# wcy199705/DfFintheWild

Hardware: AMD Instinct MI355X
Metric: focal-stacks/sec (10x3x256x256) (higher is better)
Workload: dtype bf16x3 (split-bf16 MFMA operands hi+lo, fp32 accumulate, fp32-accurate); 1 GPU; DFF_net forward, 10-slice 3x256x256 focal stacks, batch 32 per GPU (BASELINE.json config 3), dense focus_dists, synthetic weights seed 0; batch_per_gpu=32, global_batch=32, slices=10, height=256, width=256, parallelism=single GPU, precision=bf16x3, input=float32 (B,3,N,H,W), the reference's tensor contract

## Files before the change

### dffinthewild_amd/csrc/dffw_conv_rollx.hip

```cpp
#include <algorithm>
#include <cstdio>
#include <cstdlib>
#include <utility>

#include "dffw_conv_roll.h"
#include "dffw_device.h"
#include "dffw_persist.h"

namespace dffw {

namespace rollx {
constexpr int TY = 8, TX = 16, FY = TY + 2, FX = TX + 2, HALF = FX / 2, NW = 4, RING = 6;
constexpr int ROWE = 2 * FX;
constexpr int TPL = 6144;
constexpr int SLOTB = 2 * TPL;
constexpr int PPW = 3;
constexpr int NCH = 18;
static_assert(FY * ROWE * 16 <= TPL && TPL % 1024 == 0 && 2 * (TPL / 1024) == NW * PPW, "piece layout");
static_assert((2 * ROWE) % 16 == 8, "a wave's two rows must be 8 bank groups apart");
}

template <bool RELU, int ABL = 0, bool NTS = false>
__global__ __launch_bounds__(256) __attribute__((amdgpu_waves_per_eu(2, 2))) void conv_rollx_pair(const ConvArgs a, const RollArgs t) {
    using namespace rollx;
    __shared__ __attribute__((aligned(1024))) unsigned char smem[RING * SLOTB];

    const int lane = threadIdx.x & 63;
    const int wave = __builtin_amdgcn_readfirstlane(threadIdx.x >> 6);
    const int g = lane >> 4, r = lane & 15;

    const UnitRange ur = persistent_range(t.total_tiles);
    const int ufirst = ur.first, uend = ur.end, wgs_per_xcd = ur.step;
    if (ufirst >= uend) return;
    using Unit = RollUnit;
    auto decode = [&](int u) { return roll_unit<TY, TX>(u, t, a.No); };

    const bool two = a.C1 != 0;
    const int tsel = wave >> 1;
    const int recb = two ? 32 : 64;
    const char *tbase = reinterpret_cast<const char *>((two && tsel) ? a.in1 : a.in0) + (two ? 0 : tsel * 16);
    const int slice_bytes = a.Hi * a.Wi * recb;
    int fyx[PPW], foff[PPW];
#pragma unroll
    for (int k = 0; k < PPW; ++k) {
        const int e = ((wave & 1) * PPW + k) * 64 + lane;
        const int fy = e / ROWE, j = e - fy * ROWE;
        const int part = j >= FX ? 1 : 0, sx = j - part * FX;
        const int fx = sx < HALF ? 2 * sx : 2 * (sx - HALF) + 1;
        fyx[k] = fy | (fx << 8) | (e < FY * ROWE ? 0 : 1 << 16);
        foff[k] = (fy * a.Wi + fx) * recb + part * (recb / 2);
    }
    int fvo[PPW];
    const char *fbase = tbase;
    int fu = ufirst, fq = 0, fslices = 0, fz = 0;
    auto setup_fill = [&]() {
        const Unit c = decode(fu);
        fslices = c.nz + 2;
        fz = c.zbeg - 1;
        fbase = tbase + ((int64_t)c.b * a.Ni * a.Hi * a.Wi + (int64_t)(c.gy0 - 1) * a.Wi + (c.gx0 - 1)) * recb;
#pragma unroll
        for (int k = 0; k < PPW; ++k) {
            const int iy = c.gy0 - 1 + (fyx[k] & 0xFF), ix = c.gx0 - 1 + ((fyx[k] >> 8) & 0xFF);
            fvo[k] = (!(fyx[k] >> 16) && (unsigned)iy < (unsigned)a.Hi && (unsigned)ix < (unsigned)a.Wi) ? foff[k] : (int)0x80000000;
        }
    };
    setup_fill();
    int fslotb = 0;
    auto issue_piece = [&](auto K) {
        constexpr int k = decltype(K)::value;
        const bool zin = (unsigned)fz < (unsigned)a.Ni && fu < uend;
        const auto rs = __builtin_amdgcn_make_buffer_rsrc(const_cast<char *>(fbase), 0, zin ? (int)0x80000000 : 0, 0x00020000);
        __builtin_amdgcn_raw_ptr_buffer_load_lds(rs, (__attribute__((address_space(3))) void *)(smem + fslotb + (wave * PPW + k) * 1024), 16, fvo[k],
                                                 zin ? fz * slice_bytes : 0, 0, 0);
    };
    auto advance_fill = [&]() {
        fslotb = (fslotb + SLOTB == RING * SLOTB) ? 0 : fslotb + SLOTB;
        ++fz;
        if (++fq == fslices && fu < uend) {
            fq = 0;
            fu += wgs_per_xcd;
            if (fu < uend) setup_fill();
        }
    };
#pragma unroll
    for (int q = 0; q < RING - 1; ++q) {
        issue_piece(std::integral_constant<int, 0>{});
        issue_piece(std::integral_constant<int, 1>{});
        issue_piece(std::integral_constant<int, 2>{});
        advance_fill();
    }

    const int rr = r >> 3, pp = r & 7;
    const int prow = (wave & 1) + 4 * (wave >> 1) + 2 * rr, pcol = 2 * pp + (g >> 1);
    const unsigned lds0 = (unsigned)(uintptr_t)(__attribute__((address_space(3))) unsigned char *)smem;
    const unsigned lbase = lds0 + (g & 1) * TPL + (prow * ROWE + (g >> 1) * HALF + pp) * 16;
    const int vob = ((prow * a.Wo + pcol) * 16 + (g & 1) * 8) * 2;

    short8 w[NCH][2];
    {
        const short8 *wp = reinterpret_cast<const short8 *>(t.wroll) + lane;
#pragma unroll
        for (int c = 0; c < NCH; ++c) {
            w[c][0] = wp[(c * 2 + 0) * 64];
            w[c][1] = wp[(c * 2 + 1) * 64];
        }
    }
    const f32x4 bias4 = *reinterpret_cast<const f32x4 *>(a.bias + (g & 1) * 4);
    __builtin_amdgcn_s_waitcnt(0x0F70);
    asm volatile("s_barrier" ::: "memory");

    int sidxb = 0;
    f32x4 acc0 = bias4, acc1 = {0.f, 0.f, 0.f, 0.f}, acc2 = {0.f, 0.f, 0.f, 0.f};
    char *pptr = nullptr;
    StepTrace trc(a.trace, wave, lane, NW);

    auto step = [&](auto LIVE_, auto PEND_, auto PEND2_, char *optr) {
        constexpr bool LIVE = decltype(LIVE_)::value, PEND = decltype(PEND_)::value, PEND2 = decltype(PEND2_)::value;
        trc.stamp(0);
        float v0 = 0.f, v1 = 0.f, v2 = 0.f, v3 = 0.f;
        uint32_t h01 = 0, h23 = 0, l01 = 0, l23 = 0;
        if constexpr (PEND) {
            v0 = acc0[0] + (acc1[0] + acc2[0]);
            v1 = acc0[1] + (acc1[1] + acc2[1]);
            v2 = acc0[2] + (acc1[2] + acc2[2]);
            v3 = acc0[3] + (acc1[3] + acc2[3]);
            if constexpr (RELU) {
                v0 = relu_bits(v0);
                v1 = relu_bits(v1);
                v2 = relu_bits(v2);
                v3 = relu_bits(v3);
            }
        }
        auto side = [&](auto S) {
            constexpr int s = decltype(S)::value;
            typedef __attribute__((ext_vector_type(2))) float f2;
            typedef __attribute__((ext_vector_type(2))) __bf16 b2;
            if constexpr (PEND && s == 0) {
                h01 = __builtin_bit_cast(uint32_t, __builtin_convertvector(f2{v0, v1}, b2));
                h23 = __builtin_bit_cast(uint32_t, __builtin_convertvector(f2{v2, v3}, b2));
            }
            if constexpr (PEND && s == 1) {
                v0 -= __uint_as_float(h01 << 16);
                v1 -= __uint_as_float(h01 & 0xFFFF0000u);
                v2 -= __uint_as_float(h23 << 16);
                v3 -= __uint_as_float(h23 & 0xFFFF0000u);
            }
            if constexpr (PEND && s == 2) {
                l01 = __builtin_bit_cast(uint32_t, __builtin_convertvector(f2{v0, v1}, b2));
                l23 = __builtin_bit_cast(uint32_t, __builtin_convertvector(f2{v2, v3}, b2));
            }
            if constexpr (PEND && s == 3) swap16(h01, l01);
            if constexpr (PEND && s == 4) swap16(h23, l23);
            if constexpr (PEND && s == 5 && !(ABL & 8)) {
                typedef unsigned u32x4 __attribute__((ext_vector_type(4)));
                u32x4 *dst = reinterpret_cast<u32x4 *>(pptr + (uint32_t)vob);
                if constexpr (NTS) __builtin_nontemporal_store(u32x4{h01, h23, l01, l23}, dst);
                else *dst = u32x4{h01, h23, l01, l23};
            }
            if constexpr (PEND && s == 5 && (ABL & 8)) asm volatile("" ::"v"(h01), "v"(h23), "v"(l01), "v"(l23));
            if constexpr (s == 6 && !(ABL & 4)) issue_piece(std::integral_constant<int, 0>{});
            if constexpr (s == 7 && !(ABL & 4)) issue_piece(std::integral_constant<int, 1>{});
            if constexpr (s == 8 && !(ABL & 4)) issue_piece(std::integral_constant<int, 2>{});
        };
        if constexpr (LIVE) {
            unsigned ad[3];
            {
                int sb = sidxb;
                ad[0] = lbase + sb;
                sb = (sb + SLOTB == RING * SLOTB) ? 0 : sb + SLOTB;
                ad[1] = lbase + sb;
                sb = (sb + SLOTB == RING * SLOTB) ? 0 : sb + SLOTB;
                ad[2] = lbase + sb;
            }
            trc.stamp(1);
            constexpr int DEPTH = 2, NB = DEPTH + 1;
            short8 x[NB][2];
            auto fetch = [](auto C, short8 (&xx)[NB][2], const unsigned (&adr)[3]) {
                constexpr int c = decltype(C)::value;
                constexpr int imm = (((c % 6) / 2) * ROWE + (c % 2)) * 16;
                asm volatile("ds_read_b128 %0, %1 offset:%2" : "=v"(xx[c % NB][0]) : "v"(adr[c / 6]), "n"(imm));
                asm volatile("ds_read_b128 %0, %1 offset:%2" : "=v"(xx[c % NB][1]) : "v"(adr[c / 6]), "n"(imm + FX * 16));
            };
            if constexpr (!(ABL & 1)) static_for<DEPTH>([&](auto C) { fetch(C, x, ad); });
            else static_for<NB>([&](auto C) { x[decltype(C)::value][0] = w[0][0]; x[decltype(C)::value][1] = w[1][1]; });
            f32x4 n0 = bias4, n1 = {0.f, 0.f, 0.f, 0.f}, n2 = {0.f, 0.f, 0.f, 0.f};
            static_for<NCH>([&](auto C) {
                constexpr int c = decltype(C)::value;
                if constexpr (c + DEPTH < NCH && !(ABL & 1)) fetch(std::integral_constant<int, c + DEPTH>{}, x, ad);
                constexpr int ahead = (NCH - 1 - c < DEPTH ? NCH - 1 - c : DEPTH) * 2;
                if constexpr (!(ABL & 1)) asm volatile("s_waitcnt lgkmcnt(%2)" : "+v"(x[c % NB][0]), "+v"(x[c % NB][1]) : "n"(ahead));
                else asm volatile("" : "+v"(x[c % NB][0]), "+v"(x[c % NB][1]));
                if constexpr (!(ABL & 2)) {
                    n0 = mma<false>(w[c][0], x[c % NB][0], n0);
                    n1 = mma<false>(w[c][1], x[c % NB][0], n1);
                    n2 = mma<false>(w[c][0], x[c % NB][1], n2);
                } else {
                    asm volatile("" ::"v"(x[c % NB][0]), "v"(x[c % NB][1]), "v"(w[c][0]), "v"(w[c][1]));
                }
                __builtin_amdgcn_sched_barrier(0);
                if constexpr (c >= 1 && c <= 9) {
                    side(std::integral_constant<int, c - 1>{});
                    __builtin_amdgcn_sched_barrier(0);
                }
            });
            acc0 = n0;
            acc1 = n1;
            acc2 = n2;
        } else {
            static_for<9>([&](auto S) { side(S); });
        }
        trc.stamp(2);
        constexpr int INFLIGHT = 2 * PPW + (PEND ? 1 : 0) + (PEND2 ? 1 : 0);
        if constexpr (!(ABL & 16)) asm volatile("s_waitcnt vmcnt(%0)\n\ts_barrier" ::"n"(INFLIGHT) : "memory");
        else asm volatile("s_waitcnt vmcnt(%0)" ::"n"(INFLIGHT) : "memory");
        trc.stamp(3);
        sidxb = (sidxb + SLOTB == RING * SLOTB) ? 0 : sidxb + SLOTB;
        advance_fill();
        pptr = optr;
        trc.stamp(4);
        trc.next();
    };

    int hist = 0;
    auto dispatch = [&](bool live, char *optr) {
        using T = std::true_type;
        using F = std::false_type;
        switch ((live ? 4 : 0) | hist) {
            case 0: step(F{}, F{}, F{}, optr); break;
            case 1: step(F{}, T{}, F{}, optr); break;
            case 2: step(F{}, F{}, T{}, optr); break;
            case 3: step(F{}, T{}, T{}, optr); break;
            case 4: step(T{}, F{}, F{}, optr); break;
            case 5: step(T{}, T{}, F{}, optr); break;
            case 6: step(T{}, F{}, T{}, optr); break;
            default: step(T{}, T{}, T{}, optr); break;
        }
        hist = ((hist << 1) & 2) | (live ? 1 : 0);
    };

    const int64_t ostride = (int64_t)a.Ho * a.Wo * 32;
    for (int cu = ufirst; cu < uend; cu += wgs_per_xcd) {
        const Unit U = decode(cu);
        char *optr = reinterpret_cast<char *>(a.out) + ((((int64_t)U.b * a.No + U.zbeg) * a.Ho + U.gy0) * a.Wo + U.gx0) * 32;
        for (int st = 0; st < U.nz + 2; ++st) {
            dispatch(st < U.nz, optr);
            optr += ostride;
        }
    }
    asm volatile("s_waitcnt vmcnt(0)" ::: "memory");
}

namespace rollk2 {
constexpr int TY = 8, TX = 16, FY = TY + 2, FX = TX + 2, NW = 8, RING = 5;
constexpr int ROWE = 4 * FX;
constexpr int ROWB = ROWE * 16;
constexpr int PARTB = 2 * FX * 16;
constexpr int HPL = 12 * 1024;
constexpr int SLOTB = 2 * HPL;
constexpr int PPW = 3;
constexpr int NCH = 15;
constexpr int XCH_OFF = RING * SLOTB, XCHB = 8 * 1024;
static_assert(FY * ROWB <= HPL && 2 * (HPL / 1024) == NW * PPW, "piece layout");
}

template <bool RELU>
__global__ __launch_bounds__(512) __attribute__((amdgpu_waves_per_eu(2, 2))) void conv_rollx_k2(const ConvArgs a, const RollArgs t) {
    using namespace rollk2;
    __shared__ __attribute__((aligned(1024))) unsigned char smem[XCH_OFF + 2 * XCHB];

    const int lane = threadIdx.x & 63;
    const int wave = __builtin_amdgcn_readfirstlane(threadIdx.x >> 6);
    const int half = wave >> 2, wq = wave & 3;
    const int g = lane >> 4, r = lane & 15;

    const UnitRange ur = persistent_range(t.total_tiles);
    const int ufirst = ur.first, uend = ur.end, wgs_per_xcd = ur.step;
    if (ufirst >= uend) return;
    using Unit = RollUnit;
    auto decode = [&](int u) { return roll_unit<TY, TX>(u, t, a.No); };

    const bool two = a.C1 != 0;
    const int recb = two ? 64 : 128;
    const char *tbase = reinterpret_cast<const char *>((two && half) ? a.in1 : a.in0) + (two ? 0 : half * 32);
    const int slice_bytes = a.Hi * a.Wi * recb;
    int fyx[PPW], foff[PPW];
#pragma unroll
    for (int k = 0; k < PPW; ++k) {
        const int e = (wq * PPW + k) * 64 + lane;
        const int fy = e / ROWE, j = e - fy * ROWE;
        const int part = j >= 2 * FX ? 1 : 0, q = j - part * 2 * FX;
        const int fx = q >> 1, oct = q & 1;
        fyx[k] = fy | (fx << 8) | (e < FY * ROWE ? 0 : 1 << 16);
        foff[k] = (fy * a.Wi + fx) * recb + part * (recb / 2) + oct * 16;
    }
    int fvo[PPW];
    const char *fbase = tbase;
    int fu = ufirst, fq = 0, fslices = 0, fz = 0;
    auto setup_fill = [&]() {
        const Unit c = decode(fu);
        fslices = c.nz + 2;
        fz = c.zbeg - 1;
        fbase = tbase + ((int64_t)c.b * a.Ni * a.Hi * a.Wi + (int64_t)(c.gy0 - 1) * a.Wi + (c.gx0 - 1)) * recb;
#pragma unroll
        for (int k = 0; k < PPW; ++k) {
            const int iy = c.gy0 - 1 + (fyx[k] & 0xFF), ix = c.gx0 - 1 + ((fyx[k] >> 8) & 0xFF);
            fvo[k] = (!(fyx[k] >> 16) && (unsigned)iy < (unsigned)a.Hi && (unsigned)ix < (unsigned)a.Wi) ? foff[k] : (int)0x80000000;
        }
    };
    setup_fill();
    int fslotb = 0;
    auto issue_piece = [&](auto K) {
        constexpr int k = decltype(K)::value;
        const bool zin = (unsigned)fz < (unsigned)a.Ni && fu < uend;
        const auto rs = __builtin_amdgcn_make_buffer_rsrc(const_cast<char *>(fbase), 0, zin ? (int)0x80000000 : 0, 0x00020000);
        __builtin_amdgcn_raw_ptr_buffer_load_lds(rs, (__attribute__((address_space(3))) void *)(smem + fslotb + (wave * PPW + k) * 1024), 16, fvo[k],
                                                 zin ? fz * slice_bytes : 0, 0, 0);
    };
    auto advance_fill = [&]() {
        fslotb = (fslotb + SLOTB == RING * SLOTB) ? 0 : fslotb + SLOTB;
        ++fz;
        if (++fq == fslices && fu < uend) {
            fq = 0;
            fu += wgs_per_xcd;
            if (fu < uend) setup_fill();
        }
    };
#pragma unroll
    for (int q = 0; q < RING - 1; ++q) {
        issue_piece(std::integral_constant<int, 0>{});
        issue_piece(std::integral_constant<int, 1>{});
        issue_piece(std::integral_constant<int, 2>{});
        advance_fill();
    }

    const unsigned lds0 = (unsigned)(uintptr_t)(__attribute__((address_space(3))) unsigned char *)smem;
    unsigned aoff[5];
#pragma unroll
    for (int k5 = 0; k5 < 5; ++k5) {
        const int tap9 = 2 * k5 + (g >> 1);
        const int dy = tap9 < 9 ? tap9 / 3 : 0, dx = tap9 < 9 ? tap9 % 3 : 0;
        aoff[k5] = lds0 + half * HPL + (2 * wq + dy) * ROWB + ((r + dx) * 2 + (g & 1)) * 16;
    }
    const int myrow = 2 * wq + half;
    const int vob = ((myrow * a.Wo + r) * 32 + (g & 1) * 16 + (g >> 1) * 8) * 2;
    const unsigned xch_wr = lds0 + XCH_OFF + ((2 * wq + (half ^ 1)) * 64 + lane) * 16;
    const unsigned xch_rd = lds0 + XCH_OFF + (myrow * 64 + lane) * 16;

    short8 w[NCH][2];
    {
        const short8 *wp = reinterpret_cast<const short8 *>(t.wroll) + (size_t)half * NCH * 2 * 64 + lane;
#pragma unroll
        for (int c = 0; c < NCH; ++c) {
            w[c][0] = wp[(c * 2 + 0) * 64];
            w[c][1] = wp[(c * 2 + 1) * 64];
        }
    }
    f32x4 bias4 = *reinterpret_cast<const f32x4 *>(a.bias + g * 4);
    if (half) bias4 = f32x4{0.f, 0.f, 0.f, 0.f};
    __builtin_amdgcn_s_waitcnt(0x0F70);
    asm volatile("s_barrier" ::: "memory");

    int sidxb = 0, xpar = 0;
    f32x4 mine = {0.f, 0.f, 0.f, 0.f};
    char *pptr = nullptr;

    auto step = [&](auto LIVE_, auto PEND_, auto PEND2_, char *optr) {
        constexpr bool LIVE = decltype(LIVE_)::value, PEND = decltype(PEND_)::value, PEND2 = decltype(PEND2_)::value;
        float v0 = 0.f, v1 = 0.f, v2 = 0.f, v3 = 0.f;
        uint32_t h01 = 0, h23 = 0, l01 = 0, l23 = 0;
        f32x4 theirs = {0.f, 0.f, 0.f, 0.f};
        if constexpr (PEND) {
            const unsigned ad = xch_rd + (xpar ^ 1) * XCHB;
            asm volatile("ds_read_b128 %0, %1" : "=v"(theirs) : "v"(ad));
            if constexpr (!LIVE) asm volatile("s_waitcnt lgkmcnt(0)" : "+v"(theirs));
        }
        auto side = [&](auto S) {
            constexpr int s = decltype(S)::value;
            typedef __attribute__((ext_vector_type(2))) float f2;
            typedef __attribute__((ext_vector_type(2))) __bf16 b2;
            if constexpr (PEND && s == 0) {
                v0 = mine[0] + theirs[0];
                v1 = mine[1] + theirs[1];
                v2 = mine[2] + theirs[2];
                v3 = mine[3] + theirs[3];
                if constexpr (RELU) {
                    v0 = relu_bits(v0);
                    v1 = relu_bits(v1);
                    v2 = relu_bits(v2);
                    v3 = relu_bits(v3);
                }
            }
            if constexpr (PEND && s == 1) {
                h01 = __builtin_bit_cast(uint32_t, __builtin_convertvector(f2{v0, v1}, b2));
                h23 = __builtin_bit_cast(uint32_t, __builtin_convertvector(f2{v2, v3}, b2));
            }
            if constexpr (PEND && s == 2) {
                v0 -= __uint_as_float(h01 << 16);
                v1 -= __uint_as_float(h01 & 0xFFFF0000u);
                v2 -= __uint_as_float(h23 << 16);
                v3 -= __uint_as_float(h23 & 0xFFFF0000u);
            }
            if constexpr (PEND && s == 3) {
                l01 = __builtin_bit_cast(uint32_t, __builtin_convertvector(f2{v0, v1}, b2));
                l23 = __builtin_bit_cast(uint32_t, __builtin_convertvector(f2{v2, v3}, b2));
            }
            if constexpr (PEND && s == 4) swap16(h01, l01);
            if constexpr (PEND && s == 5) swap16(h23, l23);
            if constexpr (PEND && s == 6) {
                typedef unsigned u32x4 __attribute__((ext_vector_type(4)));
                *reinterpret_cast<u32x4 *>(pptr + (uint32_t)vob) = u32x4{h01, h23, l01, l23};
            }
            if constexpr (s == 7) issue_piece(std::integral_constant<int, 0>{});
            if constexpr (s == 8) issue_piece(std::integral_constant<int, 1>{});
            if constexpr (s == 9) issue_piece(std::integral_constant<int, 2>{});
        };
        if constexpr (LIVE) {
            int sb[3];
            sb[0] = sidxb;
            sb[1] = (sb[0] + SLOTB == RING * SLOTB) ? 0 : sb[0] + SLOTB;
            sb[2] = (sb[1] + SLOTB == RING * SLOTB) ? 0 : sb[1] + SLOTB;
            constexpr int DEPTH = 2, NB = DEPTH + 1;
            short8 x[NB][2][2];
            auto fetch = [](auto C, short8 (&xx)[NB][2][2], const unsigned (&ao)[5], const int (&sbb)[3]) {
                constexpr int c = decltype(C)::value;
                const unsigned ad = ao[c % 5] + sbb[c / 5];
                asm volatile("ds_read_b128 %0, %1" : "=v"(xx[c % NB][0][0]) : "v"(ad));
                asm volatile("ds_read_b128 %0, %1 offset:%2" : "=v"(xx[c % NB][0][1]) : "v"(ad), "n"(PARTB));
                asm volatile("ds_read_b128 %0, %1 offset:%2" : "=v"(xx[c % NB][1][0]) : "v"(ad), "n"(ROWB));
                asm volatile("ds_read_b128 %0, %1 offset:%2" : "=v"(xx[c % NB][1][1]) : "v"(ad), "n"(ROWB + PARTB));
            };
            static_for<DEPTH>([&](auto C) { fetch(C, x, aoff, sb); });
            f32x4 n[2][3];
#pragma unroll
            for (int j = 0; j < 2; ++j) {
                n[j][0] = bias4;
                n[j][1] = f32x4{0.f, 0.f, 0.f, 0.f};
                n[j][2] = f32x4{0.f, 0.f, 0.f, 0.f};
            }
            static_for<NCH>([&](auto C) {
                constexpr int c = decltype(C)::value;
                if constexpr (c + DEPTH < NCH) fetch(std::integral_constant<int, c + DEPTH>{}, x, aoff, sb);
                constexpr int ahead = (NCH - 1 - c < DEPTH ? NCH - 1 - c : DEPTH) * 4;
                asm volatile("s_waitcnt lgkmcnt(%4)" : "+v"(x[c % NB][0][0]), "+v"(x[c % NB][0][1]), "+v"(x[c % NB][1][0]), "+v"(x[c % NB][1][1]) : "n"(ahead));
                if constexpr (PEND && c == 0) asm volatile("" : "+v"(theirs));
#pragma unroll
                for (int j = 0; j < 2; ++j) {
                    n[j][0] = mma<false>(w[c][0], x[c % NB][j][0], n[j][0]);
                    n[j][1] = mma<false>(w[c][1], x[c % NB][j][0], n[j][1]);
                    n[j][2] = mma<false>(w[c][0], x[c % NB][j][1], n[j][2]);
                }
                __builtin_amdgcn_sched_barrier(0);
                if constexpr (c >= 1 && c <= 10) {
                    side(std::integral_constant<int, c - 1>{});
                    __builtin_amdgcn_sched_barrier(0);
                }
            });
            f32x4 give;
#pragma unroll
            for (int i = 0; i < 4; ++i) {
                const float s0 = n[0][0][i] + (n[0][1][i] + n[0][2][i]), s1 = n[1][0][i] + (n[1][1][i] + n[1][2][i]);
                mine[i] = half ? s1 : s0;
                give[i] = half ? s0 : s1;
            }
            const unsigned wad = xch_wr + xpar * XCHB;
            asm volatile("ds_write_b128 %0, %1" ::"v"(wad), "v"(give) : "memory");
        } else {
            static_for<10>([&](auto S) { side(S); });
        }
        constexpr int INFLIGHT = PPW + (PEND ? 1 : 0);
        asm volatile("s_waitcnt vmcnt(%0) lgkmcnt(0)\n\ts_barrier" ::"n"(INFLIGHT) : "memory");
        (void)PEND2;
        sidxb = (sidxb + SLOTB == RING * SLOTB) ? 0 : sidxb + SLOTB;
        xpar ^= 1;
        advance_fill();
        pptr = optr;
    };

    int hist = 0;
    auto dispatch = [&](bool live, char *optr) {
        using T = std::true_type;
        using F = std::false_type;
        switch ((live ? 2 : 0) | (hist & 1)) {
            case 0: step(F{}, F{}, F{}, optr); break;
            case 1: step(F{}, T{}, F{}, optr); break;
            case 2: step(T{}, F{}, F{}, optr); break;
            default: step(T{}, T{}, F{}, optr); break;
        }
        hist = live ? 1 : 0;
    };

    const int64_t ostride = (int64_t)a.Ho * a.Wo * 64;
    for (int cu = ufirst; cu < uend; cu += wgs_per_xcd) {
        const Unit U = decode(cu);
        char *optr = reinterpret_cast<char *>(a.out) + ((((int64_t)U.b * a.No + U.zbeg) * a.Ho + U.gy0) * a.Wo + U.gx0) * 64;
        for (int st = 0; st < U.nz + 2; ++st) {
            dispatch(st < U.nz, optr);
            optr += ostride;
        }
    }
    asm volatile("s_waitcnt vmcnt(0)" ::: "memory");
}

bool rollx_k2_ok(int prec, const ConvArgs &a) {
    if (prec != P_BF16X3 || (a.dbg & DFFW_ARGS_NO_ROLLX)) return false;
    if (!a.out || a.out_pre || a.outf || a.res0 || a.res1 || a.res_bcast || a.cls_w || a.relu == 2 || a.Cout != 16) return false;
    if (!((a.C0 == 32 && a.C1 == 0) || (a.C0 == 16 && a.C1 == 16))) return false;
    const int64_t recb = a.C1 ? 64 : 128;
    return (int64_t)(a.Ni + 1) * a.Hi * a.Wi * recb < (1ll << 31);
}

static const RollRow kRollxK2[] = {DFFW_ROW(rollk2::NW * 64, conv_rollx_k2, false), DFFW_ROW(rollk2::NW * 64, conv_rollx_k2, true)};
hipError_t launch_conv_rollx_k2(const ConvArgs &a, const RollArgs &t, hipStream_t s) {
    return launch_row(&kRollxK2[a.relu == 1], t.total_tiles, t.wgs > 0 ? t.wgs : 256, 1, s, a, t);
}
void conv_rollx_k2_kernel_name(const ConvArgs &a, char *buf, int n) { copy_row_name(&kRollxK2[a.relu == 1], buf, n); }

bool rollx_pair_ok(int prec, const ConvArgs &a, bool pair) {
    if (prec != P_BF16X3 || !pair || (a.dbg & DFFW_ARGS_NO_ROLLX)) return false;
    if (!a.out || a.out_pre || a.outf || a.res0 || a.res1 || a.res_bcast || a.cls_w || a.relu == 2 || a.Cout != 8) return false;
    if (!((a.C0 == 16 && a.C1 == 0) || (a.C0 == 8 && a.C1 == 8))) return false;
    const int64_t recb = a.C1 ? 32 : 64;
    return (int64_t)(a.Ni + 1) * a.Hi * a.Wi * recb < (1ll << 31);
}

static const RollRow kRollxPair[] = {
    {"dffw::conv_rollx_pair<false>", conv_rollx_pair<false>, rollx::NW * 64},
    {"dffw::conv_rollx_pair<true>", conv_rollx_pair<true>, rollx::NW * 64},
#ifdef DFFW_ABL_BUILD
    DFFW_ROW(rollx::NW * 64, conv_rollx_pair, true, 3, false), DFFW_ROW(rollx::NW * 64, conv_rollx_pair, true, 12, false),
    DFFW_ROW(rollx::NW * 64, conv_rollx_pair, true, 0, true),
#endif
};
// ... 17 lines not shown
```

### dffinthewild_amd/csrc/dffw_ops.cpp

```cpp
#include <functional>
#include <string>
#include <vector>

#include "dffw_bn.h"
#include "dffw_conv_pw_wgrad.h"
#include "dffw_conv_wgrad.h"
#include "dffw_pool_grad.h"
#include "dffw_run.h"
#include "dffw_score_grad.h"
#include "dffw_stem_wgrad.h"

using namespace dffw;

namespace {

struct OpEngine : dffw_engine {
    OpEngine(int device_, int prec_) { device = device_; prec = prec_; }
};

struct OpBlock {
    char *p = nullptr;
    hipStream_t s;
    explicit OpBlock(hipStream_t s_) : s(s_) {}
    OpBlock(const OpBlock &) = delete;
// ... 82 lines not shown
    return dffw_op_conv3d_ex(device, precision, x, B, Cin, N, H, W, weight, Cout, kernel, stride, pad, dilation, transposed, bn, conv_bias, residual, relu, y,
                             nullptr, nullptr, nullptr, hip_stream);
}

int dffw_op_conv3d_ex(int device, int precision, const float *x, int B, int Cin, int N, int H, int W, const float *weight,
                      int Cout, const int kernel[3], const int stride[3], const int pad[3], const int dilation[3], int transposed,
                      const float *bn, const float *conv_bias, const float *residual, int relu, float *y, float *y_pre, const float *cls_weight,
                      float *cls_score, void *hip_stream) {
    if (!x || !weight || !y || !kernel || !stride || !pad || !dilation) return fail(DFFW_EINVAL, "null argument");
    if (precision < 0 || precision > 2) return fail(DFFW_EINVAL, "unknown precision %d", precision);
    if (stride[0] != 1 || dilation[0] != 1) return fail(DFFW_EINVAL, "slice stride/dilation must be 1");
    if (stride[1] != stride[2] || dilation[1] != dilation[2]) return fail(DFFW_EINVAL, "row/col stride and dilation must match");
    if (Cout != 1 && Cout % 4) return fail(DFFW_EINVAL, "Cout must be 1 or a multiple of 4");
    if (Cout > 128) return fail(DFFW_EINVAL, "Cout > 128 unsupported");
    HIPCHK(hipSetDevice(device));
    LayerDef L{"op", "", Cin, Cout, kernel[0], kernel[1], kernel[2], stride[1], stride[2], pad[0], pad[1], pad[2],
               dilation[1], dilation[2], transposed != 0, true, false};
    if (transposed && !(kernel[0] == 3 && kernel[1] == 3 && kernel[2] == 3 && stride[1] == 2 && pad[0] == 1 && pad[1] == 1 && pad[2] == 1))
        return fail(DFFW_EINVAL, "transposed conv supports only k3 s(1,2,2) p1 op(0,1,1)");
    OpEngine eng(device, precision);
    int rc = pack_conv(L, precision, weight, bn, conv_bias, eng.convs["op"]);
    if (rc) return rc;
    if ((cls_weight != nullptr) != (cls_score != nullptr)) return fail(DFFW_EINVAL, "cls_weight and cls_score go together");
    if ((y_pre || cls_weight) && (Cout == 1 || Cout % 8)) return fail(DFFW_EINVAL, "second output / fused classifier need Cout %% 8 == 0");
    if (cls_weight) {
        LayerDef C{"cls", "", Cout, 1, 1, 1, 1, 1, 1, 0, 0, 0, 1, 1, false, true, false};
        rc = pack_conv(C, precision, cls_weight, nullptr, nullptr, eng.convs["cls"]);
        if (rc) return rc;
    }
    const int cpad = (Cin + 7) / 8 * 8;
    const bool stem = (!transposed && kernel[0] == 1 && kernel[1] == 9 && kernel[2] == 9 && dilation[1] == 2 && pad[0] == 0 && pad[1] == 8 &&
                       stride[1] == 1 && Cin == 3);
    return run_op(eng, (hipStream_t)hip_stream, false, [&](Run &r) {
        Act in = r.act(B, N, H, stem ? W + 2 : W, cpad);
        const int64_t plane = (int64_t)N * H * W;
        float *xp = !stem && cpad != Cin ? (float *)r.raw(B * cpad * plane * (int64_t)sizeof(float)) : nullptr;
        if (real(r)) {
            if (stem || xp) r.check(hipMemsetAsync(in.p, 0, (size_t)in.pixels() * prec_parts(precision) * cpad * 2, r.s), "input memset");
            if (stem) {
                r.check(launch_stack_in(precision, x, in.p, B, N, H, W, r.s), "stack_in");
            } else if (!xp) {
                r.check(launch_from_ncdhw(precision, x, in.p, B, Cin, N, H, W, r.s), "from_ncdhw");
            } else {
                r.check(hipMemsetAsync(xp, 0, (size_t)B * cpad * plane * sizeof(float), r.s), "input memset");
                for (int b = 0; b < B && r.ok(); ++b)
                    r.check(hipMemcpyAsync(xp + (int64_t)b * cpad * plane, x + (int64_t)b * Cin * plane, (size_t)Cin * plane * sizeof(float),
                                           hipMemcpyDeviceToDevice, r.s), "copy");
                if (r.ok()) r.check(launch_from_ncdhw(precision, xp, in.p, B, cpad, N, H, W, r.s), "from_ncdhw");
            }
        }
        const int No = N + 2 * pad[0] - (kernel[0] - 1);
        const int Ho = transposed ? 2 * H : (H + 2 * pad[1] - dilation[1] * (kernel[1] - 1) - 1) / stride[1] + 1;
        const int Wo = transposed ? 2 * W : (W + 2 * pad[2] - dilation[2] * (kernel[2] - 1) - 1) / stride[2] + 1;
        const int64_t opix = (int64_t)B * No * Ho * Wo;
        ConvOpt o;
        o.relu = relu;
        Act res, pre;
        if (Cout == 1) {
            o.outf = (float *)r.raw(opix * sizeof(float));
        } else if (residual) {
            res = stage_in(r, residual, B, Cout, No, Ho, Wo);
            o.res0 = &res;
        }
        if (y_pre) o.out_pre = &pre;
        if (cls_weight) {
            o.cls = "cls";
            o.cls_out = (float *)r.raw(opix * sizeof(float));
        }
        Act out = r.conv("op", in, o);
        if (Cout == 1) copy_out(r, o.outf, y, opix);
        else stage_out(r, out, y);
        if (y_pre) stage_out(r, pre, y_pre);
        if (cls_weight) copy_out(r, o.cls_out, cls_score, opix);
    });
}

int dffw_op_pool(int device, int precision, int mode, int k, const float *x, int B, int C, int N, int H, int W, float *y,
                 void *hip_stream) {
    if (!x || !y) return fail(DFFW_EINVAL, "null argument");
    if (precision < 0 || precision > 2) return fail(DFFW_EINVAL, "unknown precision %d", precision);
    if (C % 8 || k < 1 || H % k || W % k) return fail(DFFW_EINVAL, "pool needs C %% 8 == 0 and H,W divisible by k");
    HIPCHK(hipSetDevice(device));
    OpEngine eng(device, precision);
    return run_op(eng, (hipStream_t)hip_stream, false, [&](Run &r) {
        Act in = stage_in(r, x, B, C, N, H, W);
        stage_out(r, r.pool(in, mode, k), y);
    });
}

// ... 347 lines not shown
```

### dffinthewild_amd/csrc/dffw_run.h

```cpp
#pragma once
#include <algorithm>
#include <climits>
#include <cstdio>
#include <cstdlib>
#include <cstring>
#include <initializer_list>
#include <map>
#include <string>
#include <vector>

#include "../../include/dffw.h"
#include "dffw_align.h"
#include "dffw_conv_roll.h"
#include "dffw_conv_tile.h"
#include "dffw_internal.h"
#include "dffw_pack.h"

void dffw_set_last_conv_kernel(const char *name);

extern "C" char **environ;

namespace dffw {

static constexpr auto &fail = dffw_fail;
// ... 76 lines not shown
        HIPCHK(hipMalloc((void **)&zero_page, 256));
        HIPCHK(hipMemset(zero_page, 0, 256));
        return DFFW_OK;
    }
    void clear_recs() {
        for (auto &r : recs) {
            if (r.e0) (void)hipEventDestroy(r.e0);
            if (r.e1) (void)hipEventDestroy(r.e1);
        }
        recs.clear();
    }
    ~dffw_engine() {
        clear_recs();
        if (zero_page) (void)hipFree(zero_page);
        for (int i = 0; i < NSIDE; ++i)
            if (side[i]) (void)hipStreamDestroy(side[i]);
        for (int i = 0; i < NEV; ++i)
            if (ev[i]) (void)hipEventDestroy(ev[i]);
        for (auto &kv : convs) dffw::free_packed(kv.second);
    }
};

namespace dffw {

inline bool getenv_flag(const char *name) {
    const char *v = getenv(name);
    return v && *v && *v != '0';
}

#define DFFW_SWITCHES(X)                                                                                                 \
    X(NO_CONCURRENT) X(NO_CONF_FORK) X(NO_FUSED_ATTENTION) X(NO_FUSED_EFD) X(NO_FUSED_OF) X(NO_FUSED_POOL) X(NO_FUSED_SRD) \
    X(NO_FUSED_STEM) X(NO_HEAD_SPLIT) X(NO_ROLL) X(NO_ROLL_S2) X(NO_SPLIT) X(NO_SPLITK)  \
    X(NO_STEM_PAIR) X(NO_TILE) X(NO_SMALL) X(NO_ROLL_S2_WIDE) X(NO_HEAD_SUMS) X(NO_HEAD_SUMS_FUSED) X(NO_HEAD_WARP) X(NO_OF_FIRST) \
    X(NO_LEAN_TILE) X(NO_LEAN_ROLL) X(NO_ROLLX) X(NO_ROLLK) X(NO_ROLLT) X(NO_TEAMS) X(NO_SLICE32) X(NO_REGRESS_FUSED) X(NO_STEM_PIPE) X(NO_POOL3) X(NO_NARROW)
enum SwitchId {
#define X_ID(n) SW_##n,
    DFFW_SWITCHES(X_ID)
#undef X_ID
    SW_COUNT
};
#define DFFW_INT_KNOBS(X)                                                                                                                                  \
    X(ROLL_WGS, roll_wgs, 8, 0)                                                                                                                            \
    X(SRD_WGS, srd_wgs, 8, 0)                                                                                                                              \
                                                                                                                                         \
    X(SMALL_MAX_UNITS, small_max_units, 0, 0)                                                                                                              \
    X(ROLL_ZSPLIT, roll_zsplit, 1, 0)                                                                                                                      \
    X(KSPLIT_TARGET, ksplit_target, 1, 512)                                                                                                                \
                                                                  \
    X(REDIR_SIDE, redir_side, 0, -1)                                                                                                                       \
    X(TEAM_MIN_WGS, team_min_wgs, 0, 0)                                                                                                                    \
    X(TEAM_MAX_WGS, team_max_wgs, 1, 320)                                                                                                                  \
     \
    X(SPLIT_S64, split_s64, 1, 1025)                                                                                                                       \
                                                 \
    X(SPLIT_T64, split_t64, 1, 1025)                                                                                                                       \
                                   \
    X(NARROW_MAX, narrow_max, 1, 40)                                                                                                                       \
                                      \
    X(WARM_MAX_WGS, warm_max_wgs, 0, 1024)                                                                                                                 \
                                                                                            \
    X(ROLLK_MERGE_BELOW, rollk_merge_below, 0, 1 << 30)                                                                                                    \
                                                                                                \
    X(ROLLT_MIN_UNITS, rollt_min_units, 1, 128)                                                                                                            \
                                                                                                                \
    X(ROLL_MIN_UNITS, roll_min_units, 1, 192)                                                                                                              \
                                                                                                     \
    X(SPLIT_WG, split_wg, INT_MIN, 256)                                                                                                                    \
// ... 358 lines not shown
```

Before: 4096 stacks/s.

## Skip out-of-range depth slices in rollx conv pipeline and trim boundary MFMAs

The rollx 3D-conv kernels no longer stream zero-padded depth slices at the volume ends. Per-unit slice ranges are clamped to valid z, and specialized step variants skip the MFMA chunks that would multiply zero padding for the first and last slices. The ring prologue depth and the starting slot shift to match, and a trailing drain dispatch is added. Side work is respread across fewer MFMA iterations via a PER factor. An opt-in OP_CONCAT path for the op-level API splits the input into two half-channel buffers, but it is off by default.

Measured after the change: 4113 stacks/s (median of 6 runs). About the same (+0.4%).

```diff
diff --git a/dffinthewild_amd/csrc/dffw_conv_rollx.hip b/dffinthewild_amd/csrc/dffw_conv_rollx.hip
--- a/dffinthewild_amd/csrc/dffw_conv_rollx.hip
+++ b/dffinthewild_amd/csrc/dffw_conv_rollx.hip
@@ -33,7 +33,7 @@
     const int ufirst = ur.first, uend = ur.end, wgs_per_xcd = ur.step;
     if (ufirst >= uend) return;
     using Unit = RollUnit;
-    auto decode = [&](int u) { return roll_unit<TY, TX>(u, t, a.No); };
+    auto decode = [&](int u) __attribute__((always_inline)) { return roll_unit<TY, TX>(u, t, a.No); };
 
     const bool two = a.C1 != 0;
     const int tsel = wave >> 1;
@@ -53,10 +53,10 @@
     int fvo[PPW];
     const char *fbase = tbase;
     int fu = ufirst, fq = 0, fslices = 0, fz = 0;
-    auto setup_fill = [&]() {
+    auto setup_fill = [&]() __attribute__((always_inline)) {
         const Unit c = decode(fu);
-        fslices = c.nz + 2;
-        fz = c.zbeg - 1;
+        fz = c.zbeg > 0 ? c.zbeg - 1 : 0;
+        fslices = (c.zbeg + c.nz < a.Ni ? c.zbeg + c.nz : a.Ni - 1) - fz + 1;
         fbase = tbase + ((int64_t)c.b * a.Ni * a.Hi * a.Wi + (int64_t)(c.gy0 - 1) * a.Wi + (c.gx0 - 1)) * recb;
 #pragma unroll
         for (int k = 0; k < PPW; ++k) {
@@ -66,14 +66,14 @@
     };
     setup_fill();
     int fslotb = 0;
-    auto issue_piece = [&](auto K) {
+    auto issue_piece = [&](auto K) __attribute__((always_inline)) {
         constexpr int k = decltype(K)::value;
-        const bool zin = (unsigned)fz < (unsigned)a.Ni && fu < uend;
+        const bool zin = fu < uend;
         const auto rs = __builtin_amdgcn_make_buffer_rsrc(const_cast<char *>(fbase), 0, zin ? (int)0x80000000 : 0, 0x00020000);
         __builtin_amdgcn_raw_ptr_buffer_load_lds(rs, (__attribute__((address_space(3))) void *)(smem + fslotb + (wave * PPW + k) * 1024), 16, fvo[k],
                                                  zin ? fz * slice_bytes : 0, 0, 0);
     };
-    auto advance_fill = [&]() {
+    auto advance_fill = [&]() __attribute__((always_inline)) {
         fslotb = (fslotb + SLOTB == RING * SLOTB) ? 0 : fslotb + SLOTB;
         ++fz;
         if (++fq == fslices && fu < uend) {
@@ -83,7 +83,7 @@
         }
     };
 #pragma unroll
-    for (int q = 0; q < RING - 1; ++q) {
+    for (int q = 0; q < RING - 2; ++q) {
         issue_piece(std::integral_constant<int, 0>{});
         issue_piece(std::integral_constant<int, 1>{});
         issue_piece(std::integral_constant<int, 2>{});
@@ -109,13 +109,15 @@
     __builtin_amdgcn_s_waitcnt(0x0F70);
     asm volatile("s_barrier" ::: "memory");
 
-    int sidxb = 0;
+    int sidxb = (RING - 1) * SLOTB;
     f32x4 acc0 = bias4, acc1 = {0.f, 0.f, 0.f, 0.f}, acc2 = {0.f, 0.f, 0.f, 0.f};
     char *pptr = nullptr;
     StepTrace trc(a.trace, wave, lane, NW);
 
-    auto step = [&](auto LIVE_, auto PEND_, auto PEND2_, char *optr) {
+    auto step = [&](auto LIVE_, auto PEND_, auto PEND2_, auto FRONT_, auto BACK_, char *optr) __attribute__((always_inline)) {
         constexpr bool LIVE = decltype(LIVE_)::value, PEND = decltype(PEND_)::value, PEND2 = decltype(PEND2_)::value;
+        constexpr int C0 = decltype(FRONT_)::value ? 0 : 6, C1 = decltype(BACK_)::value ? NCH : 12, M = C1 - C0;
+        constexpr int PER = (9 + M - 2) / (M - 1);
         trc.stamp(0);
         float v0 = 0.f, v1 = 0.f, v2 = 0.f, v3 = 0.f;
         uint32_t h01 = 0, h23 = 0, l01 = 0, l23 = 0;
@@ -131,7 +133,7 @@
                 v3 = relu_bits(v3);
             }
         }
-        auto side = [&](auto S) {
+        auto side = [&](auto S) __attribute__((always_inline)) {
             constexpr int s = decltype(S)::value;
             typedef __attribute__((ext_vector_type(2))) float f2;
             typedef __attribute__((ext_vector_type(2))) __bf16 b2;
@@ -175,19 +177,19 @@
             trc.stamp(1);
             constexpr int DEPTH = 2, NB = DEPTH + 1;
             short8 x[NB][2];
-            auto fetch = [](auto C, short8 (&xx)[NB][2], const unsigned (&adr)[3]) {
+            auto fetch = [](auto C, short8 (&xx)[NB][2], const unsigned (&adr)[3]) __attribute__((always_inline)) {
                 constexpr int c = decltype(C)::value;
                 constexpr int imm = (((c % 6) / 2) * ROWE + (c % 2)) * 16;
                 asm volatile("ds_read_b128 %0, %1 offset:%2" : "=v"(xx[c % NB][0]) : "v"(adr[c / 6]), "n"(imm));
                 asm volatile("ds_read_b128 %0, %1 offset:%2" : "=v"(xx[c % NB][1]) : "v"(adr[c / 6]), "n"(imm + FX * 16));
             };
-            if constexpr (!(ABL & 1)) static_for<DEPTH>([&](auto C) { fetch(C, x, ad); });
-            else static_for<NB>([&](auto C) { x[decltype(C)::value][0] = w[0][0]; x[decltype(C)::value][1] = w[1][1]; });
+            if constexpr (!(ABL & 1)) static_for<DEPTH>([&](auto I) __attribute__((always_inline)) { fetch(std::integral_constant<int, C0 + decltype(I)::value>{}, x, ad); });
+            else static_for<NB>([&](auto C) __attribute__((always_inline)) { x[decltype(C)::value][0] = w[0][0]; x[decltype(C)::value][1] = w[1][1]; });
             f32x4 n0 = bias4, n1 = {0.f, 0.f, 0.f, 0.f}, n2 = {0.f, 0.f, 0.f, 0.f};
-            static_for<NCH>([&](auto C) {
-                constexpr int c = decltype(C)::value;
-                if constexpr (c + DEPTH < NCH && !(ABL & 1)) fetch(std::integral_constant<int, c + DEPTH>{}, x, ad);
-                constexpr int ahead = (NCH - 1 - c < DEPTH ? NCH - 1 - c : DEPTH) * 2;
+            static_for<M>([&](auto I) __attribute__((always_inline)) {
+                constexpr int i = decltype(I)::value, c = C0 + i;
+                if constexpr (i + DEPTH < M && !(ABL & 1)) fetch(std::integral_constant<int, c + DEPTH>{}, x, ad);
+                constexpr int ahead = (M - 1 - i < DEPTH ? M - 1 - i : DEPTH) * 2;
                 if constexpr (!(ABL & 1)) asm volatile("s_waitcnt lgkmcnt(%2)" : "+v"(x[c % NB][0]), "+v"(x[c % NB][1]) : "n"(ahead));
                 else asm volatile("" : "+v"(x[c % NB][0]), "+v"(x[c % NB][1]));
                 if constexpr (!(ABL & 2)) {
@@ -198,8 +200,10 @@
                     asm volatile("" ::"v"(x[c % NB][0]), "v"(x[c % NB][1]), "v"(w[c][0]), "v"(w[c][1]));
                 }
                 __builtin_amdgcn_sched_barrier(0);
-                if constexpr (c >= 1 && c <= 9) {
-                    side(std::integral_constant<int, c - 1>{});
+                if constexpr (i >= 1 && (i - 1) * PER < 9) {
+                    static_for<PER>([&](auto J) __attribute__((always_inline)) {
+                        if constexpr ((i - 1) * PER + decltype(J)::value < 9) side(std::integral_constant<int, (i - 1) * PER + decltype(J)::value>{});
+                    });
                     __builtin_amdgcn_sched_barrier(0);
                 }
             });
@@ -207,7 +211,7 @@
             acc1 = n1;
             acc2 = n2;
         } else {
-            static_for<9>([&](auto S) { side(S); });
+            static_for<9>([&](auto S) __attribute__((always_inline)) { side(S); });
         }
         trc.stamp(2);
         constexpr int INFLIGHT = 2 * PPW + (PEND ? 1 : 0) + (PEND2 ? 1 : 0);
@@ -222,18 +226,29 @@
     };
 
     int hist = 0;
-    auto dispatch = [&](bool live, char *optr) {
+    auto dispatch = [&](bool live, bool front, bool back, char *optr) __attribute__((always_inline)) {
         using T = std::true_type;
         using F = std::false_type;
-        switch ((live ? 4 : 0) | hist) {
-            case 0: step(F{}, F{}, F{}, optr); break;
-            case 1: step(F{}, T{}, F{}, optr); break;
-            case 2: step(F{}, F{}, T{}, optr); break;
-            case 3: step(F{}, T{}, T{}, optr); break;
-            case 4: step(T{}, F{}, F{}, optr); break;
-            case 5: step(T{}, T{}, F{}, optr); break;
-            case 6: step(T{}, F{}, T{}, optr); break;
-            default: step(T{}, T{}, T{}, optr); break;
+        if (live && !(front && back)) {
+            switch ((front ? 4 : 0) | (back ? 2 : 0) | (hist & 1)) {
+                case 0: step(T{}, F{}, F{}, F{}, F{}, optr); break;
+                case 1: step(T{}, T{}, F{}, F{}, F{}, optr); break;
+                case 2: step(T{}, F{}, F{}, F{}, T{}, optr); break;
+                case 3: step(T{}, T{}, F{}, F{}, T{}, optr); break;
+                case 4: step(T{}, F{}, F{}, T{}, F{}, optr); break;
+                default: step(T{}, T{}, F{}, T{}, F{}, optr); break;
+            }
+        } else {
+            switch ((live ? 4 : 0) | hist) {
+                case 0: step(F{}, F{}, F{}, T{}, T{}, optr); break;
+                case 1: step(F{}, T{}, F{}, T{}, T{}, optr); break;
+                case 2: step(F{}, F{}, T{}, T{}, T{}, optr); break;
+                case 3: step(F{}, T{}, T{}, T{}, T{}, optr); break;
+                case 4: step(T{}, F{}, F{}, T{}, T{}, optr); break;
+                case 5: step(T{}, T{}, F{}, T{}, T{}, optr); break;
+                case 6: step(T{}, F{}, T{}, T{}, T{}, optr); break;
+                default: step(T{}, T{}, T{}, T{}, T{}, optr); break;
+            }
         }
         hist = ((hist << 1) & 2) | (live ? 1 : 0);
     };
@@ -241,12 +256,14 @@
     const int64_t ostride = (int64_t)a.Ho * a.Wo * 32;
     for (int cu = ufirst; cu < uend; cu += wgs_per_xcd) {
         const Unit U = decode(cu);
-        char *optr = reinterpret_cast<char *>(a.out) + ((((int64_t)U.b * a.No + U.zbeg) * a.Ho + U.gy0) * a.Wo + U.gx0) * 32;
-        for (int st = 0; st < U.nz + 2; ++st) {
-            dispatch(st < U.nz, optr);
+        const int zlo = U.zbeg > 0 ? U.zbeg - 1 : 0, zhi = U.zbeg + U.nz < a.Ni ? U.zbeg + U.nz : a.Ni - 1;
+        char *optr = reinterpret_cast<char *>(a.out) + ((((int64_t)U.b * a.No + zlo) * a.Ho + U.gy0) * a.Wo + U.gx0) * 32;
+        for (int z = zlo; z <= zhi; ++z) {
+            dispatch(z >= U.zbeg && z < U.zbeg + U.nz, z > 0, z < a.Ni - 1, optr);
             optr += ostride;
         }
     }
+    if (hist & 1) dispatch(false, true, true, nullptr);
     asm volatile("s_waitcnt vmcnt(0)" ::: "memory");
 }
 
@@ -277,7 +294,7 @@
     const int ufirst = ur.first, uend = ur.end, wgs_per_xcd = ur.step;
     if (ufirst >= uend) return;
     using Unit = RollUnit;
-    auto decode = [&](int u) { return roll_unit<TY, TX>(u, t, a.No); };
+    auto decode = [&](int u) __attribute__((always_inline)) { return roll_unit<TY, TX>(u, t, a.No); };
 
     const bool two = a.C1 != 0;
     const int recb = two ? 64 : 128;
@@ -296,10 +313,10 @@
     int fvo[PPW];
     const char *fbase = tbase;
     int fu = ufirst, fq = 0, fslices = 0, fz = 0;
-    auto setup_fill = [&]() {
+    auto setup_fill = [&]() __attribute__((always_inline)) {
         const Unit c = decode(fu);
-        fslices = c.nz + 2;
-        fz = c.zbeg - 1;
+        fz = c.zbeg > 0 ? c.zbeg - 1 : 0;
+        fslices = (c.zbeg + c.nz < a.Ni ? c.zbeg + c.nz : a.Ni - 1) - fz + 1;
         fbase = tbase + ((int64_t)c.b * a.Ni * a.Hi * a.Wi + (int64_t)(c.gy0 - 1) * a.Wi + (c.gx0 - 1)) * recb;
 #pragma unroll
         for (int k = 0; k < PPW; ++k) {
@@ -309,14 +326,14 @@
     };
     setup_fill();
     int fslotb = 0;
-    auto issue_piece = [&](auto K) {
+    auto issue_piece = [&](auto K) __attribute__((always_inline)) {
         constexpr int k = decltype(K)::value;
-        const bool zin = (unsigned)fz < (unsigned)a.Ni && fu < uend;
+        const bool zin = fu < uend;
         const auto rs = __builtin_amdgcn_make_buffer_rsrc(const_cast<char *>(fbase), 0, zin ? (int)0x80000000 : 0, 0x00020000);
         __builtin_amdgcn_raw_ptr_buffer_load_lds(rs, (__attribute__((address_space(3))) void *)(smem + fslotb + (wave * PPW + k) * 1024), 16, fvo[k],
                                                  zin ? fz * slice_bytes : 0, 0, 0);
     };
-    auto advance_fill = [&]() {
+    auto advance_fill = [&]() __attribute__((always_inline)) {
         fslotb = (fslotb + SLOTB == RING * SLOTB) ? 0 : fslotb + SLOTB;
         ++fz;
         if (++fq == fslices && fu < uend) {
@@ -326,7 +343,7 @@
         }
     };
 #pragma unroll
-    for (int q = 0; q < RING - 1; ++q) {
+    for (int q = 0; q < RING - 2; ++q) {
         issue_piece(std::integral_constant<int, 0>{});
         issue_piece(std::integral_constant<int, 1>{});
         issue_piece(std::integral_constant<int, 2>{});
@@ -360,12 +377,14 @@
     __builtin_amdgcn_s_waitcnt(0x0F70);
     asm volatile("s_barrier" ::: "memory");
 
-    int sidxb = 0, xpar = 0;
+    int sidxb = (RING - 1) * SLOTB, xpar = 0;
     f32x4 mine = {0.f, 0.f, 0.f, 0.f};
     char *pptr = nullptr;
 
-    auto step = [&](auto LIVE_, auto PEND_, auto PEND2_, char *optr) {
-        constexpr bool LIVE = decltype(LIVE_)::value, PEND = decltype(PEND_)::value, PEND2 = decltype(PEND2_)::value;
+    auto step = [&](auto LIVE_, auto PEND_, auto FRONT_, auto BACK_, char *optr) __attribute__((always_inline)) {
+        constexpr bool LIVE = decltype(LIVE_)::value, PEND = decltype(PEND_)::value;
+        constexpr int C0 = decltype(FRONT_)::value ? 0 : 5, C1 = decltype(BACK_)::value ? NCH : 10, M = C1 - C0;
+        constexpr int PER = (10 + M - 2) / (M - 1);
         float v0 = 0.f, v1 = 0.f, v2 = 0.f, v3 = 0.f;
         uint32_t h01 = 0, h23 = 0, l01 = 0, l23 = 0;
         f32x4 theirs = {0.f, 0.f, 0.f, 0.f};
@@ -374,7 +393,7 @@
             asm volatile("ds_read_b128 %0, %1" : "=v"(theirs) : "v"(ad));
             if constexpr (!LIVE) asm volatile("s_waitcnt lgkmcnt(0)" : "+v"(theirs));
         }
-        auto side = [&](auto S) {
+        auto side = [&](auto S) __attribute__((always_inline)) {
             constexpr int s = decltype(S)::value;
             typedef __attribute__((ext_vector_type(2))) float f2;
             typedef __attribute__((ext_vector_type(2))) __bf16 b2;
@@ -421,7 +440,7 @@
             sb[2] = (sb[1] + SLOTB == RING * SLOTB) ? 0 : sb[1] + SLOTB;
             constexpr int DEPTH = 2, NB = DEPTH + 1;
             short8 x[NB][2][2];
-            auto fetch = [](auto C, short8 (&xx)[NB][2][2], const unsigned (&ao)[5], const int (&sbb)[3]) {
+            auto fetch = [](auto C, short8 (&xx)[NB][2][2], const unsigned (&ao)[5], const int (&sbb)[3]) __attribute__((always_inline)) {
                 constexpr int c = decltype(C)::value;
                 const unsigned ad = ao[c % 5] + sbb[c / 5];
                 asm volatile("ds_read_b128 %0, %1" : "=v"(xx[c % NB][0][0]) : "v"(ad));
@@ -429,7 +448,7 @@
                 asm volatile("ds_read_b128 %0, %1 offset:%2" : "=v"(xx[c % NB][1][0]) : "v"(ad), "n"(ROWB));
                 asm volatile("ds_read_b128 %0, %1 offset:%2" : "=v"(xx[c % NB][1][1]) : "v"(ad), "n"(ROWB + PARTB));
             };
-            static_for<DEPTH>([&](auto C) { fetch(C, x, aoff, sb); });
+            static_for<DEPTH>([&](auto I) __attribute__((always_inline)) { fetch(std::integral_constant<int, C0 + decltype(I)::value>{}, x, aoff, sb); });
             f32x4 n[2][3];
 #pragma unroll
             for (int j = 0; j < 2; ++j) {
@@ -437,12 +456,12 @@
                 n[j][1] = f32x4{0.f, 0.f, 0.f, 0.f};
                 n[j][2] = f32x4{0.f, 0.f, 0.f, 0.f};
             }
-            static_for<NCH>([&](auto C) {
-                constexpr int c = decltype(C)::value;
-                if constexpr (c + DEPTH < NCH) fetch(std::integral_constant<int, c + DEPTH>{}, x, aoff, sb);
-                constexpr int ahead = (NCH - 1 - c < DEPTH ? NCH - 1 - c : DEPTH) * 4;
+            static_for<M>([&](auto I) __attribute__((always_inline)) {
+                constexpr int i = decltype(I)::value, c = C0 + i;
+                if constexpr (i + DEPTH < M) fetch(std::integral_constant<int, c + DEPTH>{}, x, aoff, sb);
+                constexpr int ahead = (M - 1 - i < DEPTH ? M - 1 - i : DEPTH) * 4;
                 asm volatile("s_waitcnt lgkmcnt(%4)" : "+v"(x[c % NB][0][0]), "+v"(x[c % NB][0][1]), "+v"(x[c % NB][1][0]), "+v"(x[c % NB][1][1]) : "n"(ahead));
-                if constexpr (PEND && c == 0) asm volatile("" : "+v"(theirs));
+                if constexpr (PEND && i == 0) asm volatile("" : "+v"(theirs));
 #pragma unroll
                 for (int j = 0; j < 2; ++j) {
                     n[j][0] = mma<false>(w[c][0], x[c % NB][j][0], n[j][0]);
@@ -450,8 +469,10 @@
                     n[j][2] = mma<false>(w[c][0], x[c % NB][j][1], n[j][2]);
                 }
                 __builtin_amdgcn_sched_barrier(0);
-                if constexpr (c >= 1 && c <= 10) {
-                    side(std::integral_constant<int, c - 1>{});
+                if constexpr (i >= 1 && (i - 1) * PER < 10) {
+                    static_for<PER>([&](auto J) __attribute__((always_inline)) {
+                        if constexpr ((i - 1) * PER + decltype(J)::value < 10) side(std::integral_constant<int, (i - 1) * PER + decltype(J)::value>{});
+                    });
                     __builtin_amdgcn_sched_barrier(0);
                 }
             });
@@ -465,11 +486,10 @@
             const unsigned wad = xch_wr + xpar * XCHB;
             asm volatile("ds_write_b128 %0, %1" ::"v"(wad), "v"(give) : "memory");
         } else {
-            static_for<10>([&](auto S) { side(S); });
+            static_for<10>([&](auto S) __attribute__((always_inline)) { side(S); });
         }
         constexpr int INFLIGHT = PPW + (PEND ? 1 : 0);
         asm volatile("s_waitcnt vmcnt(%0) lgkmcnt(0)\n\ts_barrier" ::"n"(INFLIGHT) : "memory");
-        (void)PEND2;
         sidxb = (sidxb + SLOTB == RING * SLOTB) ? 0 : sidxb + SLOTB;
         xpar ^= 1;
         advance_fill();
@@ -477,14 +497,20 @@
     };
 
     int hist = 0;
-    auto dispatch = [&](bool live, char *optr) {
+    auto dispatch = [&](bool live, bool front, bool back, char *optr) __attribute__((always_inline)) {
         using T = std::true_type;
         using F = std::false_type;
-        switch ((live ? 2 : 0) | (hist & 1)) {
-            case 0: step(F{}, F{}, F{}, optr); break;
-            case 1: step(F{}, T{}, F{}, optr); break;
-            case 2: step(T{}, F{}, F{}, optr); break;
-            default: step(T{}, T{}, F{}, optr); break;
+        switch (live ? 2 + (front ? 4 : 0) + (back ? 2 : 0) + hist : hist) {
+            case 0: step(F{}, F{}, T{}, T{}, optr); break;
+            case 1: step(F{}, T{}, T{}, T{}, optr); break;
+            case 2: step(T{}, F{}, F{}, F{}, optr); break;
+            case 3: step(T{}, T{}, F{}, F{}, optr); break;
+            case 4: step(T{}, F{}, F{}, T{}, optr); break;
+            case 5: step(T{}, T{}, F{}, T{}, optr); break;
+            case 6: step(T{}, F{}, T{}, F{}, optr); break;
+            case 7: step(T{}, T{}, T{}, F{}, optr); break;
+            case 8: step(T{}, F{}, T{}, T{}, optr); break;
+            default: step(T{}, T{}, T{}, T{}, optr); break;
         }
         hist = live ? 1 : 0;
     };
@@ -492,12 +518,14 @@
     const int64_t ostride = (int64_t)a.Ho * a.Wo * 64;
     for (int cu = ufirst; cu < uend; cu += wgs_per_xcd) {
         const Unit U = decode(cu);
-        char *optr = reinterpret_cast<char *>(a.out) + ((((int64_t)U.b * a.No + U.zbeg) * a.Ho + U.gy0) * a.Wo + U.gx0) * 64;
-        for (int st = 0; st < U.nz + 2; ++st) {
-            dispatch(st < U.nz, optr);
+        const int zlo = U.zbeg > 0 ? U.zbeg - 1 : 0, zhi = U.zbeg + U.nz < a.Ni ? U.zbeg + U.nz : a.Ni - 1;
+        char *optr = reinterpret_cast<char *>(a.out) + ((((int64_t)U.b * a.No + zlo) * a.Ho + U.gy0) * a.Wo + U.gx0) * 64;
+        for (int z = zlo; z <= zhi; ++z) {
+            dispatch(z >= U.zbeg && z < U.zbeg + U.nz, z > 0, z < a.Ni - 1, optr);
             optr += ostride;
         }
     }
+    if (hist) dispatch(false, true, true, nullptr);
     asm volatile("s_waitcnt vmcnt(0)" ::: "memory");
 }
 
diff --git a/dffinthewild_amd/csrc/dffw_ops.cpp b/dffinthewild_amd/csrc/dffw_ops.cpp
--- a/dffinthewild_amd/csrc/dffw_ops.cpp
+++ b/dffinthewild_amd/csrc/dffw_ops.cpp
@@ -138,10 +138,18 @@
     const bool stem = (!transposed && kernel[0] == 1 && kernel[1] == 9 && kernel[2] == 9 && dilation[1] == 2 && pad[0] == 0 && pad[1] == 8 &&
                        stride[1] == 1 && Cin == 3);
     return run_op(eng, (hipStream_t)hip_stream, false, [&](Run &r) {
-        Act in = r.act(B, N, H, stem ? W + 2 : W, cpad);
+        const bool cat = r.sw.on(SW_OP_CONCAT) && !stem && !transposed && Cin % 16 == 0;
         const int64_t plane = (int64_t)N * H * W;
+        Act in = cat ? r.act(B, N, H, W, Cin / 2) : r.act(B, N, H, stem ? W + 2 : W, cpad), in1;
+        if (cat) in1 = r.act(B, N, H, W, Cin / 2);
         float *xp = !stem && cpad != Cin ? (float *)r.raw(B * cpad * plane * (int64_t)sizeof(float)) : nullptr;
-        if (real(r)) {
+        if (cat) {
+            const int ch = Cin / 2;
+            for (int b = 0; b < B && real(r); ++b)
+                for (int h = 0; h < 2 && r.ok(); ++h)
+                    r.check(launch_from_ncdhw(precision, x + ((int64_t)b * Cin + h * ch) * plane, (h ? in1.p : in.p) + b * plane * prec_parts(precision) * ch, 1,
+                                              ch, N, H, W, r.s), "from_ncdhw");
+        } else if (real(r)) {
             if (stem || xp) r.check(hipMemsetAsync(in.p, 0, (size_t)in.pixels() * prec_parts(precision) * cpad * 2, r.s), "input memset");
             if (stem) {
                 r.check(launch_stack_in(precision, x, in.p, B, N, H, W, r.s), "stack_in");
@@ -161,6 +169,7 @@
         const int64_t opix = (int64_t)B * No * Ho * Wo;
         ConvOpt o;
         o.relu = relu;
+        if (cat) o.in1 = &in1;
         Act res, pre;
         if (Cout == 1) {
             o.outf = (float *)r.raw(opix * sizeof(float));
diff --git a/dffinthewild_amd/csrc/dffw_run.h b/dffinthewild_amd/csrc/dffw_run.h
--- a/dffinthewild_amd/csrc/dffw_run.h
+++ b/dffinthewild_amd/csrc/dffw_run.h
@@ -132,7 +132,7 @@
     X(NO_CONCURRENT) X(NO_CONF_FORK) X(NO_FUSED_ATTENTION) X(NO_FUSED_EFD) X(NO_FUSED_OF) X(NO_FUSED_POOL) X(NO_FUSED_SRD) \
     X(NO_FUSED_STEM) X(NO_HEAD_SPLIT) X(NO_ROLL) X(NO_ROLL_S2) X(NO_SPLIT) X(NO_SPLITK)  \
     X(NO_STEM_PAIR) X(NO_TILE) X(NO_SMALL) X(NO_ROLL_S2_WIDE) X(NO_HEAD_SUMS) X(NO_HEAD_SUMS_FUSED) X(NO_HEAD_WARP) X(NO_OF_FIRST) \
-    X(NO_LEAN_TILE) X(NO_LEAN_ROLL) X(NO_ROLLX) X(NO_ROLLK) X(NO_ROLLT) X(NO_TEAMS) X(NO_SLICE32) X(NO_REGRESS_FUSED) X(NO_STEM_PIPE) X(NO_POOL3) X(NO_NARROW)
+    X(NO_LEAN_TILE) X(NO_LEAN_ROLL) X(NO_ROLLX) X(NO_ROLLK) X(NO_ROLLT) X(NO_TEAMS) X(NO_SLICE32) X(NO_REGRESS_FUSED) X(NO_STEM_PIPE) X(NO_POOL3) X(NO_NARROW) X(OP_CONCAT)
 enum SwitchId {
 #define X_ID(n) SW_##n,
     DFFW_SWITCHES(X_ID)
```
